# camille-004/Graph-HSCN

Hardware: AMD Instinct MI355X
Metric: graphs/sec (fwd+bwd) on Peptides-func batch=128 (higher is better)
Workload: dtype f32; 1 GPU; Graph-HSCN stage C (HSCN fwd+loss+bwd) on peptides_func-shaped graphs; graphs_per_gpu=128, global_batch=128, num_clusters=16, hidden=16, layers=3, classes=10, nodes_per_gpu=20584, ll_edges_per_gpu=41900, cluster_ids=scn_untrained, virtual_nodes_per_gpu=384, vv_edges_per_gpu=772, mode=graph, engine=resident, structure_build=per-step, steps_per_graph=15, settle=0.1 s of untimed replays before the --warmup steps

## Files before the change

### graph-hscn_amd/csrc/resident_common.h

```cpp
#pragma once
#include "hscn_common.h"

namespace {

__device__ __forceinline__ float leaky(float v, float slope) { return v > 0.f ? v : v * slope; }

typedef _Float16 half_t;
typedef _Float16 half4_t __attribute__((ext_vector_type(4)));
__device__ __forceinline__ float ldf(const float* p, size_t i) { return p[i]; }
__device__ __forceinline__ float ldf(const half_t* p, size_t i) { return (float)p[i]; }
__device__ __forceinline__ float4 ldf4(const float* p, size_t i4) { return reinterpret_cast<const float4*>(p)[i4]; }
__device__ __forceinline__ float4 ldf4(const half_t* p, size_t i4) {
  const half4_t v = reinterpret_cast<const half4_t*>(p)[i4];
  return make_float4((float)v.x, (float)v.y, (float)v.z, (float)v.w);
}
__device__ __forceinline__ void stf(float* p, size_t i, float v) { p[i] = v; }
__device__ __forceinline__ void stf(half_t* p, size_t i, float v) { p[i] = (half_t)v; }
__device__ __forceinline__ void stf4(float* p, size_t i4, float4 v) { reinterpret_cast<float4*>(p)[i4] = v; }
__device__ __forceinline__ void stf4(half_t* p, size_t i4, float4 v) {
  half4_t h;
  h.x = (half_t)v.x; h.y = (half_t)v.y; h.z = (half_t)v.z; h.w = (half_t)v.w;
  reinterpret_cast<half4_t*>(p)[i4] = h;
}
__device__ __forceinline__ void stf_sc1(float* p, size_t i, float v) {
// ... 223 lines not shown
  }
  lds_barrier();
  for (int e = G.t; e < ne; e += G.nt) {
    const int k = ek[e];
    if (k < 0) continue;
    const int p = atomicAdd(&cursor[k], -1) - 1;
    tmp[rowptr[k] + p] = e;
  }
  lds_barrier();
  for (int e = G.t; e < ne; e += G.nt) {
    const int k = ek[e];
    if (k < 0) continue;
    const int s = rowptr[k], t = rowptr[k + 1];
    int rank = 0;
    for (int q = s; q < t; ++q) rank += (tmp[q] < e) ? 1 : 0;
    col[s + rank] = eo[e];
  }
  lds_barrier();
}

constexpr int ELL_D = 6;
__device__ bool build_csr_pair_ell(const int* ek, const int* eo, int ne, int nrows, int* rowptr_a, int* col_a,
                                   int* rowptr_t, int* col_t, float* dinv, int* cnt_a, int* ell_a, int* cnt_t,
                                   int* ell_t, int* ovf, int RTn, int wave, int NWn) {
  for (int e = threadIdx.x; e < ne; e += RTn) {
    const int k = ek[e], o = eo[e];
    if (k >= 0) {
      const int pa = atomicAdd(&cnt_a[k], 1), pt = atomicAdd(&cnt_t[o], 1);
      if (pa < ELL_D) ell_a[k * ELL_D + pa] = e; else ovf[0] = 1;
      if (pt < ELL_D) ell_t[o * ELL_D + pt] = e; else ovf[0] = 1;
    }
  }
  lds_barrier();
  if (ovf[0] != 0) return false;
  const int NA = NWn > 1 ? NWn / 2 : 1;
  auto rows = [&](const int* cnt, const int* ell, const int* other, int* rowptr, int* col, float* dv, int gw, int gnw) {
    const int lane = threadIdx.x & 63, gt = gw * 64 + lane, gnt = gnw * 64;
    const int per = (nrows + gnt - 1) / gnt;
    const int wb = gw * 64 * per;
    int front = 0;
    for (int j = lane; j < wb && j < nrows; j += 64) front += cnt[j];
    front = __builtin_amdgcn_readlane(wave_incl_scan(front), 63);
    const int b = gt * per;
    int s = 0;
    for (int i = 0; i < per; ++i)
      if (b + i < nrows) s += cnt[b + i];
    int run = front + wave_incl_scan(s) - s;
    for (int i = 0; i < per; ++i) {
      const int r = b + i;
      if (r >= nrows) break;
      const int c = cnt[r];
      int ev[ELL_D];
#pragma unroll
      for (int j = 0; j < ELL_D; ++j) ev[j] = j < c ? ell[r * ELL_D + j] : 0x7fffffff;
      int ov[ELL_D];
#pragma unroll
      for (int j = 0; j < ELL_D; ++j) ov[j] = other[j < c ? ev[j] : 0];
#pragma unroll
      for (int j = 0; j < ELL_D; ++j) {
        int rank = 0;
#pragma unroll
        for (int m = 0; m < ELL_D; ++m) rank += ev[m] < ev[j] ? 1 : 0;
        if (j < c) col[run + rank] = ov[j];
      }
      rowptr[r] = run;
      if (dv) dv[r] = c > 0 ? 1.0f / sqrtf((float)c) : 0.f;
      run += c;
      if (r == nrows - 1) rowptr[nrows] = run;
    }
    if (nrows == 0 && gt == 0) rowptr[0] = 0;
  };
  if (NWn == 1) {
    rows(cnt_a, ell_a, eo, rowptr_a, col_a, dinv, 0, 1);
    rows(cnt_t, ell_t, ek, rowptr_t, col_t, nullptr, 0, 1);
  } else if (wave < NA) {
    rows(cnt_a, ell_a, eo, rowptr_a, col_a, dinv, wave, NA);
  } else {
    rows(cnt_t, ell_t, ek, rowptr_t, col_t, nullptr, wave - NA, NWn - NA);
  }
  lds_barrier();
  return true;
}

__device__ bool build_ell16_pair(const int* ek, const int* eo, int ne, int nrows, uint4* rec_a, uint4* rec_t, float* dinv,
                                 int* cnt_a, int* ell_a, int* cnt_t, int* ell_t, int* ovf, int RTn) {
  for (int e = threadIdx.x; e < ne; e += RTn) {
    const int k = ek[e], o = eo[e];
    if (k >= 0) {
      const int pa = atomicAdd(&cnt_a[k], 1), pt = atomicAdd(&cnt_t[o], 1);
      if (pa < ELL_D) ell_a[k * ELL_D + pa] = e; else ovf[0] = 1;
      if (pt < ELL_D) ell_t[o * ELL_D + pt] = e; else ovf[0] = 1;
    }
  }
  lds_barrier();
  if (ovf[0] != 0) return false;
  for (int idx = threadIdx.x; idx < 2 * nrows; idx += RTn) {
    const bool tside = idx >= nrows;
    const int r = tside ? idx - nrows : idx;
    const int* cnt = tside ? cnt_t : cnt_a;
    const int* ell = tside ? ell_t : ell_a;
    const int* other = tside ? ek : eo;
    const int c = cnt[r];
    int ev[ELL_D], ov[ELL_D];
#pragma unroll
    for (int j = 0; j < ELL_D; ++j) ev[j] = j < c ? ell[r * ELL_D + j] : 0x7fffffff;
#pragma unroll
    for (int j = 0; j < ELL_D; ++j) ov[j] = other[j < c ? ev[j] : 0];
    unsigned id[ELL_D];
#pragma unroll
    for (int j = 0; j < ELL_D; ++j) id[j] = (unsigned)r;
#pragma unroll
    for (int j = 0; j < ELL_D; ++j) {
      int rank = 0;
#pragma unroll
      for (int m = 0; m < ELL_D; ++m) rank += ev[m] < ev[j] ? 1 : 0;
#pragma unroll
      for (int q = 0; q < ELL_D; ++q)
        if (j < c && rank == q) id[q] = (unsigned)ov[j];
    }
    const uint4 rec = make_uint4(id[0] | (id[1] << 16), id[2] | (id[3] << 16), id[4] | (id[5] << 16),
                                 (unsigned)r | ((unsigned)c << 16));
    (tside ? rec_t : rec_a)[r] = rec;
    if (!tside && dinv) dinv[r] = c > 0 ? 1.0f / sqrtf((float)c) : 0.f;
  }
  lds_barrier();
  return true;
}

constexpr int CSR_MULTISPLIT_BARRIERS = 5;
__device__ void build_csr_multisplit_lds(const int* ek, const int* eo, int ne, int nrows, int* rowptr, int* col,
                                         int* cnt, int* tmp, int* wsum, const Grp& G) {
  const int nchunk = (ne + 63) >> 6;
  const int lane = threadIdx.x & 63;
  for (int i = G.t; i < nrows * nchunk; i += G.nt) cnt[i] = 0;
  lds_barrier();
  for (int c = G.w; c < nchunk; c += G.nw) {
    const int e = c * 64 + lane;
    const int k = e < ne ? ek[e] : -1;
    unsigned long long todo = __ballot(k >= 0);
    int rank = 0;
    while (todo) {
      const int leader = __ffsll((long long)todo) - 1;
      const int k0 = __builtin_amdgcn_readlane(k, leader);
      const unsigned long long m = __ballot(k == k0);
      if (k == k0) rank = __popcll(m & ((1ull << lane) - 1ull));
      if (lane == leader) cnt[k0 * nchunk + c] = __popcll(m);
      todo &= ~m;
    }
    if (e < ne) tmp[e] = rank;
  }
  lds_barrier();
  scan_inclusive_lds(cnt, nrows * nchunk, wsum, G);
  for (int r = G.t; r <= nrows; r += G.nt) rowptr[r] = (r * nchunk > 0) ? cnt[r * nchunk - 1] : 0;
  for (int e = G.t; e < ne; e += G.nt) {
    const int k = ek[e];
    if (k < 0) continue;
    const int idx = k * nchunk + (e >> 6);
    const int base = idx > 0 ? cnt[idx - 1] : 0;
    col[base + tmp[e]] = eo[e];
  }
  lds_barrier();
}

__device__ __forceinline__ void dinv_from_rowptr(const int* rowptr, int n, float* dinv, const Grp& G) {
  for (int i = G.t; i < n; i += G.nt) {
    const int d = rowptr[i + 1] - rowptr[i];
    dinv[i] = d > 0 ? 1.0f / sqrtf((float)d) : 0.f;
  }
}


template <bool ACQ>
__device__ __forceinline__ bool wait_published(const uint32_t* word, uint32_t want, int32_t* flag) {
  bool ok = true;
  if ((threadIdx.x & 63) == 0) {
    unsigned spins = 0;
// ... 74 lines not shown
```

### graph-hscn_amd/csrc/resident_kernels.h

```cpp
#pragma once
#include "hscn_common.h"
#include "resident_common.h"
#include <cstdio>

namespace {

constexpr int RT_MAX = 1024;
constexpr int MAXL = 8;

struct LayerP {
  const float *W_ll, *b_ll, *W_vv, *b_vv, *W_src, *W_dst, *att_src, *att_dst, *b_gat;
};

struct StepVCaps {
  static constexpr int N = 448, V = 32, EVV = V * (V + 1) / 2;
};

struct StepLCaps {
  static constexpr int N = 448, ELL = 1024, L = 3, C = 16;
};

struct FwdArgs {
  const float* x_local;
  const float* x_virtual;
// ... 141 lines not shown
      float d = 0.f;
#pragma unroll
      for (int q = 0; q < OPT; ++q) d = fmaf(acc[q], at[q], d);
#pragma unroll
      for (int off = LPR >> 1; off > 0; off >>= 1) d += __shfl_xor(d, off, 64);
      if (og == 0) a_out[i] = d;
    }
  }
}

template <int H>
__device__ void att_logits(const float* X, const float* Wt, const float* att, float* a_out, int n, const Grp& G) {
  constexpr int LPR = H / 4;
  constexpr int RPW = 64 / LPR;
  const int lane = threadIdx.x & 63, q = lane % LPR, rl = lane / LPR;
  if (G.w * RPW >= n) return;
  constexpr int P = 64 / H, OW = H / P;
  float wk = 0.f;
  {
    const int k = lane % H, part = lane / H;
#pragma unroll
    for (int o4 = 0; o4 < OW / 4; ++o4) {
      const float4 at = *reinterpret_cast<const float4*>(att + part * OW + 4 * o4);
      const float4 wr = *reinterpret_cast<const float4*>(Wt + k * H + part * OW + 4 * o4);
      wk = fmaf(at.w, wr.w, fmaf(at.z, wr.z, fmaf(at.y, wr.y, fmaf(at.x, wr.x, wk))));
    }
#pragma unroll
    for (int off = H; off < 64; off <<= 1) wk += __shfl_xor(wk, off, 64);
  }
  float w[4];
#pragma unroll
  for (int c = 0; c < 4; ++c) w[c] = __shfl(wk, 4 * q + c, 64);
  for (int i0 = G.w * RPW; i0 < n; i0 += G.nw * RPW) {
    const int i = i0 + rl;
    float d = 0.f;
    if (i < n) {
      const float4 x = *reinterpret_cast<const float4*>(X + i * H + 4 * q);
      d = fmaf(x.w, w[3], fmaf(x.z, w[2], fmaf(x.y, w[1], x.x * w[0])));
    }
#pragma unroll
    for (int off = LPR >> 1; off > 0; off >>= 1) d += __shfl_xor(d, off, 64);
    if (q == 0 && i < n) a_out[i] = d;
  }
}

template <int H, bool MASK>
__device__ void lin_mfma(const float* X, const float* Wt, float* Y, int n, const float* M, const Grp& G) {
  typedef float f32x4 __attribute__((ext_vector_type(4)));
  constexpr int TD = H / 16, KS = H / 4;
  const int lane = threadIdx.x & 63, li = lane & 15, lj = lane >> 4;
  const int ntile = (n + 15) >> 4;
  if (G.w >= ntile) return;
  float b[TD][KS];
#pragma unroll
  for (int ct = 0; ct < TD; ++ct)
#pragma unroll
    for (int s = 0; s < KS; ++s) b[ct][s] = Wt[(4 * s + lj) * H + ct * 16 + li];
  for (int rt = G.w; rt < ntile; rt += G.nw) {
    const int r0 = rt * 16;
    const bool ok = r0 + li < n;
    const float* xr = X + (r0 + li) * H + lj;
    f32x4 acc[TD];
#pragma unroll
    for (int ct = 0; ct < TD; ++ct) acc[ct] = f32x4{0.f, 0.f, 0.f, 0.f};
#pragma unroll
    for (int s = 0; s < KS; ++s) {
      const float a = ok ? xr[4 * s] : 0.f;
#pragma unroll
      for (int ct = 0; ct < TD; ++ct) acc[ct] = __builtin_amdgcn_mfma_f32_16x16x4f32(a, b[ct][s], acc[ct], 0, 0, 0);
    }
#pragma unroll
    for (int ct = 0; ct < TD; ++ct)
#pragma unroll
      for (int r = 0; r < 4; ++r) {
        const int row = r0 + lj * 4 + r;
        if (row < n) {
          const int idx = row * H + ct * 16 + li;
          Y[idx] = MASK ? (M[idx] > 0.f ? acc[ct][r] : 0.f) : acc[ct][r];
        }
      }
  }
}

template <int H, typename TS, bool E16 = false>
__device__ void gcn_fused(const int* rowptr, const int* col, const float* dinv, const float* X, const float* Wt,
                          const float* bias, float* Y, TS* __restrict__ gout, int n, const Grp& G,
                          float* pool_part = nullptr, float* pos_part = nullptr) {
  typedef float f32x4 __attribute__((ext_vector_type(4)));
  constexpr int TD = H / 16, KS = H / 4;
  const int lane = threadIdx.x & 63, li = lane & 15, lj = lane >> 4;
  const int ntile = (n + 15) >> 4;
  if (G.w >= ntile) {
    if (pool_part && lj == 0) {
#pragma unroll
      for (int ct = 0; ct < TD; ++ct) {
        pool_part[ct * 16 + li] = 0.f;
        if (pos_part) pos_part[ct * 16 + li] = 0.f;
      }
    }
    return;
  }
  float ps[TD], pc[TD];
#pragma unroll
  for (int ct = 0; ct < TD; ++ct) { ps[ct] = 0.f; pc[ct] = 0.f; }
  float b[TD][KS], bia[TD];
#pragma unroll
  for (int ct = 0; ct < TD; ++ct) {
    bia[ct] = bias[ct * 16 + li];
#pragma unroll
    for (int s = 0; s < KS; ++s) b[ct][s] = Wt[(KS * lj + s) * H + ct * 16 + li];
  }
  const float* xq = X + KS * lj;
  auto finish = [&](int rt_, const float (&z)[KS]) {
    const int r0 = rt_ * 16;
    f32x4 acc[TD];
#pragma unroll
    for (int ct = 0; ct < TD; ++ct) acc[ct] = f32x4{0.f, 0.f, 0.f, 0.f};
#pragma unroll
    for (int s = 0; s < KS; ++s)
#pragma unroll
      for (int ct = 0; ct < TD; ++ct) acc[ct] = __builtin_amdgcn_mfma_f32_16x16x4f32(z[s], b[ct][s], acc[ct], 0, 0, 0);
#pragma unroll
    for (int ct = 0; ct < TD; ++ct)
#pragma unroll
      for (int r = 0; r < 4; ++r) {
        const int row = r0 + lj * 4 + r;
        if (row < n) {
          const int idx = row * H + ct * 16 + li;
          const float v = rnd<TS>(fmaxf(acc[ct][r] + bia[ct], 0.f));
          Y[idx] = v;
          if (gout) stf(gout, (size_t)idx, v);
          ps[ct] += v;
          pc[ct] += v > 0.f ? 1.f : 0.f;
        }
      }
  };
  for (int rt = G.w; rt < ntile; rt += G.nw) {
    const int i = rt * 16 + li;
    float z[KS];
#pragma unroll
    for (int s = 0; s < KS; ++s) z[s] = 0.f;
    if (E16) {
      if (i < n) {
        const uint4 rec = reinterpret_cast<const uint4*>(rowptr)[i];
        const float di = dinv[i];
        const int c = (int)(rec.w >> 16);
        const int jr[8] = {(int)(rec.x & 0xffffu), (int)(rec.x >> 16), (int)(rec.y & 0xffffu), (int)(rec.y >> 16),
                           (int)(rec.z & 0xffffu), (int)(rec.z >> 16), (int)(rec.w & 0xffffu), (int)(rec.w & 0xffffu)};
#pragma unroll
        for (int p = 0; p < 8; p += 4) {
          if (p < c) {
            float w[4];
#pragma unroll
            for (int u = 0; u < 4; ++u) w[u] = p + u < c ? dinv[jr[p + u]] * di : 0.f;
#pragma unroll
            for (int q = 0; q < KS / 4; ++q) {
              float4 v[4];
#pragma unroll
              for (int u = 0; u < 4; ++u) v[u] = *reinterpret_cast<const float4*>(xq + jr[p + u] * H + 4 * q);
#pragma unroll
              for (int u = 0; u < 4; ++u) {
                z[4 * q + 0] = fmaf(w[u], v[u].x, z[4 * q + 0]);
                z[4 * q + 1] = fmaf(w[u], v[u].y, z[4 * q + 1]);
                z[4 * q + 2] = fmaf(w[u], v[u].z, z[4 * q + 2]);
                z[4 * q + 3] = fmaf(w[u], v[u].w, z[4 * q + 3]);
              }
            }
          }
        }
      }
    } else if (i < n) {
      const int s0 = rowptr[i], t0 = rowptr[i + 1];
      const float di = dinv[i];
      for (int p = s0; p < t0; p += 4) {
        int j[4];
        float w[4];
#pragma unroll
        for (int u = 0; u < 4; ++u) j[u] = col[p + u < t0 ? p + u : t0 - 1];
#pragma unroll
        for (int u = 0; u < 4; ++u) w[u] = p + u < t0 ? dinv[j[u]] * di : 0.f;
#pragma unroll
        for (int q = 0; q < KS / 4; ++q) {
          float4 v[4];
#pragma unroll
          for (int u = 0; u < 4; ++u) v[u] = *reinterpret_cast<const float4*>(xq + j[u] * H + 4 * q);
#pragma unroll
          for (int u = 0; u < 4; ++u) {
            z[4 * q + 0] = fmaf(w[u], v[u].x, z[4 * q + 0]);
            z[4 * q + 1] = fmaf(w[u], v[u].y, z[4 * q + 1]);
            z[4 * q + 2] = fmaf(w[u], v[u].z, z[4 * q + 2]);
            z[4 * q + 3] = fmaf(w[u], v[u].w, z[4 * q + 3]);
          }
        }
      }
    }
    finish(rt, z);
  }
  if (pool_part) {
#pragma unroll
    for (int ct = 0; ct < TD; ++ct) {
      float t = ps[ct];
      t += __shfl_xor(t, 16, 64);
      t += __shfl_xor(t, 32, 64);
      if (lj == 0) pool_part[ct * 16 + li] = t;
      if (pos_part) {
        float c = pc[ct];
        c += __shfl_xor(c, 16, 64);
        c += __shfl_xor(c, 32, 64);
        if (lj == 0) pos_part[ct * 16 + li] = c;
      }
    }
  }
}

template <int H>
struct Blk {
  static constexpr int OPT = H <= 16 ? 2 : 1;
};

template <int H, typename TS = float>
__device__ void agg_gcn_lds(const int* rowptr, const int* col, const float* dr, const float* dc,
                            const float* Hin, const float* bias, float* Out, int n, int relu,
                            TS* __restrict__ gout , const Grp& G) {
  constexpr int LPR = H / 4;
  const int RPB = G.nt / LPR;
  const int rl = G.t / LPR, f = (G.t % LPR) * 4;
  float4 b = make_float4(0.f, 0.f, 0.f, 0.f);
  if (bias) b = *reinterpret_cast<const float4*>(bias + f);
  for (int i = rl; i < n; i += RPB) {
    const int s = rowptr[i], t = rowptr[i + 1];
    const float di = dr[i];
    float4 a = make_float4(0.f, 0.f, 0.f, 0.f);
    for (int p = s; p < t; ++p) {
      const int j = col[p];
      const float w = mul_rn(dc[j], di);
      const float4 v = *reinterpret_cast<const float4*>(Hin + j * H + f);
      a.x = add_rn(a.x, mul_rn(w, v.x));
      a.y = add_rn(a.y, mul_rn(w, v.y));
      a.z = add_rn(a.z, mul_rn(w, v.z));
      a.w = add_rn(a.w, mul_rn(w, v.w));
    }
    a.x += b.x; a.y += b.y; a.z += b.z; a.w += b.w;
    if (relu) {
      a.x = fmaxf(a.x, 0.f); a.y = fmaxf(a.y, 0.f); a.z = fmaxf(a.z, 0.f); a.w = fmaxf(a.w, 0.f);
    }
    if (gout) { a.x = rnd<TS>(a.x); a.y = rnd<TS>(a.y); a.z = rnd<TS>(a.z); a.w = rnd<TS>(a.w); }
    *reinterpret_cast<float4*>(Out + i * H + f) = a;
    if (gout) stf4(gout, ((size_t)i * H + f) >> 2, a);
  }
}

struct FwdLayout {
  size_t xa, bh, xva, xvb, zs, a_s, a_d, sc, dinv, dinv_v, wt, headw, part, vec;
  size_t rowptr, col, rowptr_lv, col_lv, rowptr_vv, col_vv, cursorA, tmpA, cursorB, tmpB, wsum;
  size_t rowptr_t, col_t, cursorT, tmpT, cursorV, tmpV;
  size_t ck_tab, ck_first, ck_arrive, gpart;
  size_t ek_ll, eo_ll, ek_lv, eo_lv, ek_vv, eo_vv, total;
};
__host__ __device__ inline FwdLayout fwd_layout(int H, int C, int max_n, int max_v, int max_ell, int max_evv,
                                                int db, int exp) {
  FwdLayout Y;
  size_t o = 0;
  auto take = [&](size_t n) { size_t r = o; o += (n + 3) & ~(size_t)3; return r; };
  Y.xa = take((size_t)max_n * H);
  size_t xq = Y.xa;
  const size_t xend = Y.xa + (size_t)max_n * H;
  auto scratch = [&](size_t n) {
    const size_t need = (n + 3) & ~(size_t)3;
    if (xq + need <= xend) { const size_t r = xq; xq += need; return r; }
    return take(n);
  };
  const size_t stage = (size_t)2 * (((size_t)max_ell + 3) / 4 * 4 + ((size_t)max_n + 3) / 4 * 4 +
                                    ((size_t)max_evv + 3) / 4 * 4);
  const size_t two = (size_t)max_n * H;
  const size_t region = take(two > stage ? two : stage);
  Y.bh = region;
  {
    size_t p = region;
    auto sub = [&](size_t n) { size_t r = p; p += (n + 3) & ~(size_t)3; return r; };
    Y.ek_ll = sub(max_ell); Y.eo_ll = sub(max_ell);
    Y.ek_lv = sub(max_n);   Y.eo_lv = sub(max_n);
    Y.ek_vv = sub(max_evv); Y.eo_vv = sub(max_evv);
  }
  Y.xva = take((size_t)max_v * H);
  Y.xvb = take((size_t)max_v * H);
  Y.zs = take(max_v ? (size_t)(RT_MAX / 64) * H : 0);
  Y.a_s = take(max_n);
  Y.a_d = take(max_v);
  Y.sc = take(max_n);
  Y.dinv = take(max_n);
  Y.dinv_v = take(max_v);
  Y.wt = take((size_t)(db ? 2 : 1) * (4 * H * H + 5 * H));
  Y.headw = take((size_t)H * H + H + (size_t)C * H + C);
  Y.part = take((size_t)(RT_MAX / 64) * H);
  Y.vec = take(128);
// ... 1842 lines not shown
```

### graph-hscn_amd/csrc/resident_step.h

```cpp

struct StepArgs {
  const float* x_local;
  const int64_t *ll_src, *ll_dst;
  const int32_t *lptr, *eptr_ll;
  const float* W_ll[MAXL];
  const float* b_ll[MAXL];
  const float *W1, *b1, *W2, *b2;
  const float* target;
  float *pred, *score;
  float* partials;
  float* acts;
  uint32_t* ready;
  const uint32_t* epoch;
  const int32_t *pre_rp_d, *pre_col_d, *pre_rp_s, *pre_col_s;
  const float* pre_dinv;
  int32_t* flag;
  int64_t N;
  int F, L, C, head_act, max_n, max_ell, P, Pn, loss_kind;
  float inv_count;
  int B;
};

struct StepLayout {
  size_t A, dinv, wt, headw, part, vec, red, rowptr, col, rowptr_t, col_t, wsum, total;
// ... 150 lines not shown
#pragma unroll
  for (int i = 0; i < XPT; ++i) {
    const int idx = threadIdx.x + i * RT;
    const int r = idx / H, k = idx - r * H;
    const bool ok = idx < n * H && k < F;
    xr[i] = 0.f;
    if (wbase + i * RT < n * H) {
      const float t = ldf(xl_g, ok ? (size_t)(n0 + r) * F + k : 0);
      xr[i] = ok ? t : 0.f;
    }
  }
  float wr[WPT];
  const int WTOT = L * WL;
#pragma unroll
  for (int i = 0; i < WPT; ++i) {
    const int d = threadIdx.x + i * RT;
    const int l = d / WL, q = d - l * WL;
    const int fin = l == 0 ? F : H;
    wr[i] = 0.f;
    if (wbase + i * RT < WTOT) {
      const bool inb = d < WTOT;
      const int ll = inb ? l : 0;
      const bool isb = q >= H * H;
      const int k = q / H, o = q - k * H;
      const bool ok = inb && (isb || k < fin);
      const float* src = isb ? A.b_ll[ll] + (q - H * H) : A.W_ll[ll] + (ok ? o * fin + k : 0);
      const float t = *(ok ? src : A.b_ll[0]);
      wr[i] = ok ? t : 0.f;
    }
  }
  const int HT = H * H + H + C * H + C;
  auto haddr = [&](int idx) -> const float* {
    if (idx < H * H) return A.W1 + idx;
    idx -= H * H;
    if (idx < H) return A.b1 + idx;
    idx -= H;
    if (idx < C * H) return A.W2 + idx;
    idx -= C * H;
    if (idx < C) return A.b2 + idx;
    idx -= C;
    return A.target + (size_t)g * C + (idx < C ? idx : 0);
  };
  const int HTT = HT + C;
  float hw0 = *haddr((int)threadIdx.x < HTT ? (int)threadIdx.x : 0);
  float hw1 = *haddr((int)threadIdx.x + RT < HTT ? (int)threadIdx.x + RT : 0);
  if (pre) {
#pragma unroll
    for (int i = 0; i < EPT; ++i) {
      const int e = threadIdx.x + i * RT;
      if (e <= n) { rowptr[e] = prd[i]; rowptr_t[e] = prs[i]; }
      if (e < n) dinv[e] = pdv[i];
      if (e < ne) { col[e] = pcd[i]; col_t[e] = pcs[i]; }
    }
    for (int e = threadIdx.x + EPT * RT; e <= n; e += RT) {
      rowptr[e] = A.pre_rp_d[(size_t)n0 + g + e];
      rowptr_t[e] = A.pre_rp_s[(size_t)n0 + g + e];
      if (e < n) dinv[e] = A.pre_dinv[(size_t)n0 + e];
    }
    for (int e = threadIdx.x + EPT * RT; e < ne; e += RT) {
      col[e] = A.pre_col_d[(size_t)e0 + e];
      col_t[e] = A.pre_col_s[(size_t)e0 + e];
    }
  } else {
    int *ek = ib + Y.ek, *eo = ib + Y.eo;
    bool bad = false;
#pragma unroll
    for (int i = 0; i < EPT; ++i) {
      const int e = threadIdx.x + i * RT;
      if (e < ne) {
        int k = (int)(rld[i] - n0), o_ = (int)(rls[i] - n0);
        if (k < 0 || k >= n || o_ < 0 || o_ >= n) { bad = true; k = -1; o_ = -1; }
        ek[e] = k; eo[e] = o_;
      }
    }
    for (int e = threadIdx.x + EPT * RT; e < ne; e += RT) {
      int k = (int)(A.ll_dst[e0 + e] - n0), o_ = (int)(A.ll_src[e0 + e] - n0);
      if (k < 0 || k >= n || o_ < 0 || o_ >= n) { bad = true; k = -1; o_ = -1; }
      ek[e] = k; eo[e] = o_;
    }
    if (bad && A.flag) atomicOr(A.flag, 2);
  }
  for (int i = threadIdx.x; i <= n; i += RT) { (ib + Y.cntA)[i] = 0; (ib + Y.cntT)[i] = 0; }
  if (threadIdx.x == 0) { (ib + Y.wsum)[0] = 0; (ib + Y.wsum)[1] = 0; (ib + Y.ovf)[0] = 0; }
  {
    float* x0 = buf(0);
#pragma unroll
    for (int i = 0; i < XPT; ++i) {
      const int idx = threadIdx.x + i * RT;
      if (idx < n * H) x0[idx] = xr[i];
    }
    for (int idx = threadIdx.x + XPT * RT; idx < n * H; idx += RT) {
      const int r = idx / H, k = idx - r * H;
      x0[idx] = k < F ? ldf(xl_g, (size_t)(n0 + r) * F + k) : 0.f;
    }
#pragma unroll
    for (int i = 0; i < WPT; ++i) {
      const int d = threadIdx.x + i * RT;
      if (d < WTOT) wt[d] = wr[i];
    }
    for (int d = threadIdx.x + WPT * RT; d < WTOT; d += RT) {
      const int l = d / WL, q = d - l * WL;
      const int fin = l == 0 ? F : H;
      const int k = q / H, o = q - k * H;
      wt[d] = q >= H * H ? A.b_ll[l][q - H * H] : (k < fin ? A.W_ll[l][o * fin + k] : 0.f);
    }
    if ((int)threadIdx.x < HTT) headw[threadIdx.x] = hw0;
    if ((int)threadIdx.x + RT < HTT) headw[threadIdx.x + RT] = hw1;
    for (int idx = threadIdx.x + 2 * RT; idx < HTT; idx += RT) headw[idx] = *haddr(idx);
  }
  lds_barrier();
  STAMP(1);
  bool e16 = false;
  if (!pre) {
    bool low;
    if (H == 16) {
      low = build_ell16_pair(ib + Y.ek, ib + Y.eo, ne, n, reinterpret_cast<uint4*>(ib + Y.rowptr),
                             reinterpret_cast<uint4*>(ib + Y.recT), dinv, ib + Y.cntA, ib + Y.ellA, ib + Y.cntT,
                             ib + Y.ellT, ib + Y.ovf, RT);
      e16 = low;
    } else {
      low = build_csr_pair_ell(ib + Y.ek, ib + Y.eo, ne, n, rowptr, col, rowptr_t, col_t, dinv, ib + Y.cntA,
                               ib + Y.ellA, ib + Y.cntT, ib + Y.ellT, ib + Y.ovf, RT, wave, NW);
    }
    if (!low) {
      const int NA = NW / 2 > 0 ? NW / 2 : 1;
      const bool inB = wave >= NA && NW > 1;
      if (NW == 1) {
        build_csr_lds(ib + Y.ek, ib + Y.eo, ne, n, rowptr, col, ib + Y.cursorA, ib + Y.tmpA, ALL, true);
        build_csr_lds(ib + Y.eo, ib + Y.ek, ne, n, rowptr_t, col_t, ib + Y.cursorT, ib + Y.tmpT, ALL, true);
        dinv_from_rowptr(rowptr, n, dinv, ALL);
      } else if (!inB) {
        const Grp GA{(int)threadIdx.x, NA * 64, wave, NA};
        build_csr_lds(ib + Y.ek, ib + Y.eo, ne, n, rowptr, col, ib + Y.cursorA, ib + Y.tmpA, GA, true);
        dinv_from_rowptr(rowptr, n, dinv, GA);
      } else {
        const Grp GB{(int)threadIdx.x - NA * 64, (NW - NA) * 64, wave - NA, NW - NA};
        build_csr_lds(ib + Y.eo, ib + Y.ek, ne, n, rowptr_t, col_t, ib + Y.cursorT, ib + Y.tmpT, GB, true);
      }
    }
  }
  lds_barrier();
  STAMP(3);
  const bool hand = acts_g != nullptr && L >= 2;
  constexpr int NE = NW >= 16 ? 2 : 1;
  const int NC = hand && NW > 1 ? NW - NE : NW;
  const Grp GC{(int)threadIdx.x, NC * 64, wave, NC};
  auto export_rows = [&](const float* src, TS* dst) {
    typedef unsigned int u32x4 __attribute__((ext_vector_type(4)));
    typedef unsigned int u32x2 __attribute__((ext_vector_type(2)));
    const int cnt = n * (H / 4);
    const __amdgpu_buffer_rsrc_t rs = __builtin_amdgcn_make_buffer_rsrc(dst, 0, cnt * 4 * (int)sizeof(TS), 0x00020000);
    const int ew = NW > 1 ? wave - NC : 0, nes = NW > 1 ? NE : 1;
    for (int i0 = ew * 64 + lane; i0 < cnt; i0 += 4 * nes * 64) {
      float4 v[4];
#pragma unroll
      for (int u = 0; u < 4; ++u) {
        const int i = i0 + u * nes * 64;
        v[u] = reinterpret_cast<const float4*>(src)[i < cnt ? i : i0];
      }
#pragma unroll
      for (int u = 0; u < 4; ++u) {
        const int i = i0 + u * nes * 64;
        if (i >= cnt) continue;
        if constexpr (sizeof(TS) == 4) {
          u32x4 w = {__float_as_uint(v[u].x), __float_as_uint(v[u].y), __float_as_uint(v[u].z), __float_as_uint(v[u].w)};
          __builtin_amdgcn_raw_buffer_store_b128(w, rs, i * 16, 0, 16 );
        } else {
          half4_t h;
          h.x = (half_t)v[u].x; h.y = (half_t)v[u].y; h.z = (half_t)v[u].z; h.w = (half_t)v[u].w;
          u32x2 w;
          __builtin_memcpy(&w, &h, 8);
          __builtin_amdgcn_raw_buffer_store_b64(w, rs, i * 8, 0, 16 );
        }
      }
    }
  };
  int* exp_cnt = ib + Y.wsum + 1;
  auto raise = [&](int upto) {
    asm volatile("s_waitcnt vmcnt(0)" ::: "memory");
    int last = 1;
    if (NE > 1 && NW > 1) {
      int arrived = 0;
      if (lane == 0) arrived = __hip_atomic_fetch_add(exp_cnt, 1, __ATOMIC_ACQ_REL, __HIP_MEMORY_SCOPE_WORKGROUP);
      arrived = __builtin_amdgcn_readfirstlane(arrived);
      last = (arrived % NE) == NE - 1;
    }
    if (last && A.ready && lane == 0)
      __hip_atomic_store(A.ready + g, ep8 + (uint32_t)upto, __ATOMIC_RELAXED, __HIP_MEMORY_SCOPE_AGENT);
  };
  for (int l = 0; l < L; ++l) {
    STAMP(4 + l);
    float* pool_w = l == L - 1 ? partp + wave * H : nullptr;
    float* pos_w = l == L - 1 ? partp + NW * H + wave * H : nullptr;
    if (wave < NC) {
      if (e16) gcn_fused<H, TS, true>(rowptr, col, dinv, buf(l), wt + l * WL, wt + l * WL + H * H, buf(l + 1), (TS*)nullptr, n, GC, pool_w, pos_w);
      else gcn_fused<H, TS, false>(rowptr, col, dinv, buf(l), wt + l * WL, wt + l * WL + H * H, buf(l + 1), (TS*)nullptr, n, GC, pool_w, pos_w);
    } else if (hand) {
      if (pool_w && lane < H) { pool_w[lane] = 0.f; if (pos_w) pos_w[lane] = 0.f; }
      if (l >= 2) raise(l - 1);
      if (l >= 1) export_rows(buf(l), acts_g + ((size_t)(l - 1) * A.N + n0) * H);
    }
    lds_barrier();
  }
  if (hand && NW == 1) {
    for (int l = 1; l < L; ++l) export_rows(buf(l), acts_g + ((size_t)(l - 1) * A.N + n0) * H);
    raise(L - 1);
  }
  STAMP(12);
  float* aL = buf(L);
  float* pol = vec;
  float* zz = vec + 64;
  float* gz = vec + 128;
  float* gpool = vec + 192;
  float* gpn = vec + 256;
  const float* W1l = headw;
  const float* b1l = headw + H * H;
  const float* W2l = b1l + H;
  const float* b2l = W2l + C * H;
  const float* tgl = b2l + C;
  float* gpl = headw + HT + C;
  float* ltl = gpl + C;
  const bool fast_head = H == 16 && C <= 16;
  if (threadIdx.x < 64) {
    const float cnt = (float)(n > 0 ? n : 1);
    if (fast_head) {
      constexpr int HH = H <= 16 ? H : 16;
      const bool lh = lane < HH, lc = lane < C;
      const int lk = lh ? lane : 0, lcc = lc ? lane : 0;
      float pw[NW], w1r[HH], w1c[HH], w2r[HH], w2c[16];
#pragma unroll
      for (int w = 0; w < NW; ++w) pw[w] = partp[w * H + lk];
#pragma unroll
      for (int k4 = 0; k4 < HH / 4; ++k4) {
        const float4 a = *reinterpret_cast<const float4*>(W1l + lk * H + 4 * k4);
        w1r[4 * k4] = a.x; w1r[4 * k4 + 1] = a.y; w1r[4 * k4 + 2] = a.z; w1r[4 * k4 + 3] = a.w;
        const float4 b = *reinterpret_cast<const float4*>(W2l + lcc * H + 4 * k4);
        w2r[4 * k4] = b.x; w2r[4 * k4 + 1] = b.y; w2r[4 * k4 + 2] = b.z; w2r[4 * k4 + 3] = b.w;
      }
#pragma unroll
      for (int o = 0; o < HH; ++o) w1c[o] = W1l[o * H + lk];
#pragma unroll
      for (int c = 0; c < 16; ++c) w2c[c] = c < C ? W2l[c * H + lk] : 0.f;
      const float bb1 = b1l[lk], bb2 = b2l[lcc], tgt = tgl[lcc];
      float s = 0.f;
#pragma unroll
      for (int w = 0; w < NW; ++w) s += pw[w];
      const float polv = s / cnt;
      const float zv = apply_act(row_dot<HH>(polv, w1r, 0.f) + bb1, A.head_act);
      const float pc = row_dot<HH>(zv, w2r, 0.f) + bb2;
      float lt, sg, gg;
      criterion_elem(A.loss_kind, pc, tgt, A.inv_count, lt, sg, gg);
      if (lc) {
        A.pred[(size_t)g * C + lane] = pc;
        if (A.score) A.score[(size_t)g * C + lane] = sg;
      }
      lt = lc ? lt : 0.f;
      gg = lc ? gg : 0.f;
      const float sl = row_seq_sum<16>(lt, 0.f);
      const float gzv = row_dot<16>(gg, w2c, 0.f) * act_grad_from_output(zv, A.head_act);
      const float gpa = row_dot<HH>(gzv, w1c, 0.f);
      if (lh) { pol[lane] = polv; zz[lane] = zv; gz[lane] = gzv; gpool[lane] = gpa; gpn[lane] = gpa / cnt; }
      if (lc) gpl[lane] = gg;
      if (lane == 0) part[A.Pn] = sl;
    } else {
    if (lane < H) {
      float s = 0.f;
#pragma unroll
      for (int w = 0; w < NW; ++w) s += partp[w * H + lane];
      s = s / cnt;
      pol[lane] = s;
    }
    __builtin_amdgcn_fence(__ATOMIC_SEQ_CST, "wavefront");
    if (lane < H) {
      float a1 = 0.f;
      const float4* wrow = reinterpret_cast<const float4*>(W1l + lane * H);
#pragma unroll
      for (int k4 = 0; k4 < H / 4; ++k4) {
        const float4 w4 = wrow[k4];
        const float4 p4 = *reinterpret_cast<const float4*>(pol + 4 * k4);
        a1 = fmaf(p4.x, w4.x, a1);
        a1 = fmaf(p4.y, w4.y, a1);
        a1 = fmaf(p4.z, w4.z, a1);
        a1 = fmaf(p4.w, w4.w, a1);
      }
      a1 += b1l[lane];
      a1 = apply_act(a1, A.head_act);
      zz[lane] = a1;
    }
    __builtin_amdgcn_fence(__ATOMIC_SEQ_CST, "wavefront");
    for (int c = lane; c < C; c += 64) {
      float a2 = 0.f;
      const float4* wrow = reinterpret_cast<const float4*>(W2l + c * H);
#pragma unroll
      for (int k4 = 0; k4 < H / 4; ++k4) {
        const float4 w4 = wrow[k4];
        const float4 z4 = *reinterpret_cast<const float4*>(zz + 4 * k4);
        a2 = fmaf(z4.x, w4.x, a2);
        a2 = fmaf(z4.y, w4.y, a2);
        a2 = fmaf(z4.z, w4.z, a2);
        a2 = fmaf(z4.w, w4.w, a2);
      }
      const float pc = a2 + b2l[c];
      float lt, sg, gg;
      criterion_elem(A.loss_kind, pc, tgl[c], A.inv_count, lt, sg, gg);
      gpl[c] = gg;
      ltl[c] = lt;
      A.pred[(size_t)g * C + c] = pc;
      if (A.score) A.score[(size_t)g * C + c] = sg;
    }
    __builtin_amdgcn_fence(__ATOMIC_SEQ_CST, "wavefront");
    if (lane < H) {
      float acc = 0.f;
      for (int c = 0; c < C; ++c) acc = fmaf(gpl[c], W2l[c * H + lane], acc);
      gz[lane] = acc * act_grad_from_output(zz[lane], A.head_act);
    }
    __builtin_amdgcn_fence(__ATOMIC_SEQ_CST, "wavefront");
    if (lane < H) {
      float acc = 0.f;
#pragma unroll
      for (int o = 0; o < H; ++o) acc = fmaf(gz[o], W1l[o * H + lane], acc);
      gpool[lane] = acc;
      gpn[lane] = acc / cnt;
    }
    }
  }
  lds_barrier();
  STAMP(13);
  if (hand && wave >= NC && NW > 1) raise(L - 1);

  int off_head = 0;
  for (int l = 0; l < L; ++l) off_head += H * (l == 0 ? F : H) + H;
  const int oW1 = off_head, ob1 = oW1 + H * H, oW2 = ob1 + H, ob2 = oW2 + C * H;
  for (int idx = threadIdx.x; idx < C * H; idx += RT) {
    const int c = idx / H, k = idx - c * H;
    part[oW2 + idx] = gpl[c] * zz[k];
  }
  for (int c = threadIdx.x; c < C; c += RT) part[ob2 + c] = gpl[c];
  if (!fast_head && threadIdx.x == RT - 64) {
    float sl = 0.f;
    for (int c = 0; c < C; ++c) sl += ltl[c];
    part[A.Pn] = sl;
  }
  for (int idx = threadIdx.x; idx < H * H; idx += RT) {
    const int o = idx / H, k = idx - o * H;
    part[oW1 + idx] = gz[o] * pol[k];
  }
  if (threadIdx.x < H) part[ob1 + threadIdx.x] = gz[threadIdx.x];
  float* G = aL;
  float* GH = L >= 2 ? buf(0) : buf(2);
  if constexpr (H != 16) {
    const float cnt = (float)(n > 0 ? n : 1);
    for (int idx = threadIdx.x; idx < n * H; idx += RT) G[idx] = G[idx] > 0.f ? gpool[idx % H] / cnt : 0.f;
  }
  STAMP(14);
  float* bred = partp;
  constexpr int GW_TD = H / 16, GW_NT = GW_TD * GW_TD;
  constexpr int GW_TPP = GW_NT < NW ? GW_NT : NW, GW_RG = NW / GW_TPP;
  constexpr bool GW1 = GW_NT <= NW;
  auto fold_gw = [&](int t0, int oW_, int fin_) {
    for (int idx = threadIdx.x; idx < GW_TPP * 256; idx += RT) {
      const int t_ = t0 + idx / 256, e_ = idx & 255;
      if (t_ < GW_NT) {
        float s_ = 0.f;
#pragma unroll
        for (int r = 0; r < GW_RG; ++r) s_ += red[(r * GW_TPP + idx / 256) * 256 + e_];
        const int oo = (t_ / GW_TD) * 16 + (e_ >> 4), kk = (t_ % GW_TD) * 16 + (e_ & 15);
        if (kk < fin_) part[oW_ + oo * fin_ + kk] = s_;
      }
    }
  };
  int pend_oW = -1, pend_fin = 0;
  int off = off_head;
  if constexpr (H == 16) {
    typedef float f32x4 __attribute__((ext_vector_type(4)));
    int* fold_cnt = ib + Y.wsum;
    constexpr int NFW = NW < 4 ? NW : 4;
    float* Gc = aL;
    const int li = lane & 15, lj = lane >> 4;
    const int ntile = (n + 15) >> 4;
    int pend_ob = 0;
    const float4 gq4 = *reinterpret_cast<const float4*>(gpn + 4 * lj);
    auto gl4 = [](const float4 a, const float4 q) {
      return make_float4(a.x > 0.f ? q.x : 0.f, a.y > 0.f ? q.y : 0.f, a.z > 0.f ? q.z : 0.f, a.w > 0.f ? q.w : 0.f);
    };
    for (int it = 0, l = L - 1; l >= 0; --l, ++it) {
      const int fin = l == 0 ? F : H;
      off -= H * fin + H;
      const int oW = off, ob = off + H * fin;
      float* bredw = bred + (it % 3) * NW * H;
      float* bredn = bred + ((it + 1) % 3) * NW * H;
      float bsum = 0.f;
      if (it > 0) lds_barrier();
      if (pend_oW >= 0) {
        const int ft = (int)threadIdx.x - (RT - NFW * 64);
        if (ft >= 0) {
          const int e_ = ft & 255;
          float s_ = 0.f;
#pragma unroll
          for (int r = 0; r < NW; ++r) s_ += red[r * 256 + e_];
          const int oo = e_ >> 4, kk = e_ & 15;
          if (kk < pend_fin) part[pend_oW + oo * pend_fin + kk] = s_;
        }
        if ((int)threadIdx.x >= RT - H) {
          const int c_ = (int)threadIdx.x - (RT - H);
          const float* bp = bred + ((it - 1) % 3) * NW * H;
          float sb = 0.f;
#pragma unroll
          for (int w = 0; w < NW; ++w) sb += bp[w * H + c_];
          part[pend_ob + c_] = sb;
        }
        if (wave >= NW - NFW) {
          __builtin_amdgcn_fence(__ATOMIC_RELEASE, "workgroup");
          if (lane == 0) __hip_atomic_fetch_add(fold_cnt, 1, __ATOMIC_RELAXED, __HIP_MEMORY_SCOPE_WORKGROUP);
        }
      }
      if (it == 0) {
        if (lane < H) bredw[wave * H + lane] = (partp + NW * H)[wave * H + lane] * gpn[lane];
      }
      float* Xl = buf(l);
      const float* Wl = wt + l * WL;
      float bw[4];
#pragma unroll
      for (int s = 0; s < 4; ++s) bw[s] = l > 0 ? Wl[li * H + 4 * lj + s] : 0.f;
      f32x4 accw = {0.f, 0.f, 0.f, 0.f};
      float* sc = (it == 0 ? red : aL) + wave * 256;
      const float* gq = Gc + 4 * lj;
      auto finish = [&](int rt_, const float4 z) {
        const int r0 = rt_ * 16;
        __builtin_amdgcn_fence(__ATOMIC_SEQ_CST, "wavefront");
        *reinterpret_cast<float4*>(sc + li * 16 + 4 * lj) = z;
        f32x4 acc = {0.f, 0.f, 0.f, 0.f};
        if (l > 0) {
          acc = __builtin_amdgcn_mfma_f32_16x16x4f32(z.x, bw[0], acc, 0, 0, 0);
          acc = __builtin_amdgcn_mfma_f32_16x16x4f32(z.y, bw[1], acc, 0, 0, 0);
          acc = __builtin_amdgcn_mfma_f32_16x16x4f32(z.z, bw[2], acc, 0, 0, 0);
          acc = __builtin_amdgcn_mfma_f32_16x16x4f32(z.w, bw[3], acc, 0, 0, 0);
        }
        __builtin_amdgcn_fence(__ATOMIC_SEQ_CST, "wavefront");
#pragma unroll
        for (int c = 0; c < 4; ++c) {
          const int row = r0 + 4 * c + lj;
          const float av = sc[(4 * c + lj) * 16 + li];
          const float bv = row < n ? Xl[row * H + li] : 0.f;
          accw = __builtin_amdgcn_mfma_f32_16x16x4f32(av, bv, accw, 0, 0, 0);
        }
        if (l > 0) {
          __builtin_amdgcn_fence(__ATOMIC_SEQ_CST, "wavefront");
#pragma unroll
          for (int r = 0; r < 4; ++r) {
            const int row = r0 + lj * 4 + r;
            if (row < n) {
              const int idx = row * H + li;
              const float gnew = Xl[idx] > 0.f ? acc[r] : 0.f;
              Xl[idx] = gnew;
              bsum += gnew;
            }
          }
        }
      };
      for (int rt = wave; rt < ntile; rt += NW) {
        const int i = rt * 16 + li;
        float4 z = make_float4(0.f, 0.f, 0.f, 0.f);
        if (e16) {
          if (i < n) {
            const uint4 rec = reinterpret_cast<const uint4*>(ib + Y.recT)[i];
            const float di = dinv[i];
            const int c = (int)(rec.w >> 16);
            const int jr[8] = {(int)(rec.x & 0xffffu), (int)(rec.x >> 16), (int)(rec.y & 0xffffu), (int)(rec.y >> 16),
                               (int)(rec.z & 0xffffu), (int)(rec.z >> 16), (int)(rec.w & 0xffffu), (int)(rec.w & 0xffffu)};
#pragma unroll
            for (int p = 0; p < 8; p += 4) {
              if (p < c) {
                float ww[4];
                float4 vv[4];
#pragma unroll
                for (int u = 0; u < 4; ++u) {
                  ww[u] = mul_rn(dinv[jr[p + u]], di);
                  vv[u] = *reinterpret_cast<const float4*>(gq + jr[p + u] * H);
                  if (it == 0) vv[u] = gl4(vv[u], gq4);
                }
#pragma unroll
                for (int u = 0; u < 4; ++u) {
                  if (p + u < c) {
                    z.x = fmaf(ww[u], vv[u].x, z.x); z.y = fmaf(ww[u], vv[u].y, z.y);
                    z.z = fmaf(ww[u], vv[u].z, z.z); z.w = fmaf(ww[u], vv[u].w, z.w);
                  }
                }
              }
            }
          }
        } else if (i < n) {
          const int s0 = rowptr_t[i], t0 = rowptr_t[i + 1];
          const float di = dinv[i];
          for (int p = s0; p < t0; p += 4) {
            int jj[4];
            float ww[4];
            float4 vv[4];
#pragma unroll
            for (int u = 0; u < 4; ++u) jj[u] = col_t[p + u < t0 ? p + u : t0 - 1];
#pragma unroll
            for (int u = 0; u < 4; ++u) {
              ww[u] = mul_rn(dinv[jj[u]], di);
              vv[u] = *reinterpret_cast<const float4*>(gq + jj[u] * H);
              if (it == 0) vv[u] = gl4(vv[u], gq4);
            }
#pragma unroll
            for (int u = 0; u < 4; ++u) {
              if (p + u < t0) {
                z.x = fmaf(ww[u], vv[u].x, z.x); z.y = fmaf(ww[u], vv[u].y, z.y);
                z.z = fmaf(ww[u], vv[u].z, z.z); z.w = fmaf(ww[u], vv[u].w, z.w);
              }
            }
          }
        }
        finish(rt, z);
      }
      if (it > 0) {
        while (__hip_atomic_load(fold_cnt, __ATOMIC_RELAXED, __HIP_MEMORY_SCOPE_WORKGROUP) < it * NFW)
          __builtin_amdgcn_s_sleep(1);
        __builtin_amdgcn_fence(__ATOMIC_ACQUIRE, "workgroup");
      }
      __builtin_amdgcn_fence(__ATOMIC_SEQ_CST, "wavefront");
#pragma unroll
      for (int r = 0; r < 4; ++r) red[wave * 256 + (lj * 4 + r) * 16 + li] = accw[r];
      if (l > 0) {
        bsum += __shfl_xor(bsum, 16, 64);
        bsum += __shfl_xor(bsum, 32, 64);
        if (lj == 0) bredn[wave * H + li] = bsum;
      }
      pend_oW = oW; pend_fin = fin; pend_ob = ob;
      Gc = Xl;
      STAMP(16 + 3 * l);
    }
    lds_barrier();
    fold_gw(0, pend_oW, pend_fin);
    if (threadIdx.x < H) {
      const float* bp = bred + ((L - 1) % 3) * NW * H;
      float sb = 0.f;
#pragma unroll
      for (int w = 0; w < NW; ++w) sb += bp[w * H + threadIdx.x];
      part[pend_ob + threadIdx.x] = sb;
    }
    STAMP(61);
    return;
  }
  for (int l = L - 1; l >= 0; --l) {
    const int fin = l == 0 ? F : H;
    off -= H * fin + H;
    const int oW = off, ob = off + H * fin;
    lds_barrier();
    if (GW1 && pend_oW >= 0) fold_gw(0, pend_oW, pend_fin);
    const bool reload = l == 0 && L >= 2;
    float* X = reload ? buf(1) : buf(l);
    float xq[XPT];
    if (reload) {
#pragma unroll
      for (int i = 0; i < XPT; ++i) {
        const int idx = threadIdx.x + i * RT;
        const int r = idx / H, k = idx - r * H;
        xq[i] = (idx < n * H && k < fin) ? ldf(xl_g, (size_t)(n0 + r) * fin + k) : 0.f;
      }
    }
    {
      constexpr int LQ = H / 4;
      constexpr int SQ = 64 / LQ;
      const int slot = lane / LQ, f = (lane % LQ) * 4;
      float4 acc = make_float4(0.f, 0.f, 0.f, 0.f);
      for (int i = wave * SQ + slot; i < n; i += NW * SQ) {
        const float4 v = *reinterpret_cast<const float4*>(G + i * H + f);
        acc.x += v.x; acc.y += v.y; acc.z += v.z; acc.w += v.w;
      }
#pragma unroll
      for (int o_ = 32; o_ >= 16 && o_ >= LQ; o_ >>= 1) {
        acc.x += __shfl_xor(acc.x, o_, 64);
        acc.y += __shfl_xor(acc.y, o_, 64);
        acc.z += __shfl_xor(acc.z, o_, 64);
        acc.w += __shfl_xor(acc.w, o_, 64);
      }
      if (LQ <= 8) {
        acc.x = row_ror_add<8>(acc.x); acc.y = row_ror_add<8>(acc.y);
        acc.z = row_ror_add<8>(acc.z); acc.w = row_ror_add<8>(acc.w);
      }
      if (LQ <= 4) {
        acc.x = row_ror_add<4>(acc.x); acc.y = row_ror_add<4>(acc.y);
        acc.z = row_ror_add<4>(acc.z); acc.w = row_ror_add<4>(acc.w);
      }
      if (slot == 0) *reinterpret_cast<float4*>(bred + wave * H + f) = acc;
    }
    agg_gcn_lds<H, float>(rowptr_t, col_t, dinv, dinv, G, nullptr, GH, n, 0, (float*)nullptr, ALL);
    if (reload) {
#pragma unroll
      for (int i = 0; i < XPT; ++i) {
        const int idx = threadIdx.x + i * RT;
        if (idx < n * H) X[idx] = xq[i];
      }
      for (int idx = threadIdx.x + XPT * RT; idx < n * H; idx += RT) {
        const int r = idx / H, k = idx - r * H;
        X[idx] = k < fin ? ldf(xl_g, (size_t)(n0 + r) * fin + k) : 0.f;
      }
    }
    lds_barrier();
    STAMP(16 + 3 * l);
    if (threadIdx.x < H) {
      float sb = 0.f;
#pragma unroll
      for (int w = 0; w < NW; ++w) sb += bred[w * H + threadIdx.x];
      part[ob + threadIdx.x] = sb;
    }
    {
      typedef float f32x4 __attribute__((ext_vector_type(4)));
      constexpr int TD = GW_TD, NT = GW_NT, TPP = GW_TPP, RG = GW_RG;
      const int li = lane & 15, lj = lane >> 4;
// ... 103 lines not shown
```

Baseline: 5.195 million graphs/s.

## Prefetch GCN weights and ELL row records ahead of barriers in resident step

Splits gcn_fused into operand-staging and body pieces so each wave can load its layer weights, bias and first-tile ELL neighbour weights before the barrier that precedes the layer. The next layer's operands are staged right after the current one finishes. Feature/weight parking is moved into the structure build, between the atomic ELL fill and its barrier, and a redundant barrier is dropped after a successful build. Backward weights and transposed row records are also preloaded before the head and between layers. The aim is to hide global/LDS load latency behind barriers, at the cost of more registers held live.

```diff
diff --git a/graph-hscn_amd/csrc/resident_common.h b/graph-hscn_amd/csrc/resident_common.h
--- a/graph-hscn_amd/csrc/resident_common.h
+++ b/graph-hscn_amd/csrc/resident_common.h
@@ -329,8 +329,10 @@
   return true;
 }
 
-__device__ bool build_ell16_pair(const int* ek, const int* eo, int ne, int nrows, uint4* rec_a, uint4* rec_t, float* dinv,
-                                 int* cnt_a, int* ell_a, int* cnt_t, int* ell_t, int* ovf, int RTn) {
+template <typename Mid>
+__device__ __forceinline__ bool build_ell16_pair(const int* ek, const int* eo, int ne, int nrows, uint4* rec_a, uint4* rec_t,
+                                                 float* dinv, int* cnt_a, int* ell_a, int* cnt_t, int* ell_t, int* ovf,
+                                                 int RTn, Mid&& mid) {
   for (int e = threadIdx.x; e < ne; e += RTn) {
     const int k = ek[e], o = eo[e];
     if (k >= 0) {
@@ -339,6 +341,7 @@
       if (pt < ELL_D) ell_t[o * ELL_D + pt] = e; else ovf[0] = 1;
     }
   }
+  mid();
   lds_barrier();
   if (ovf[0] != 0) return false;
   for (int idx = threadIdx.x; idx < 2 * nrows; idx += RTn) {
diff --git a/graph-hscn_amd/csrc/resident_kernels.h b/graph-hscn_amd/csrc/resident_kernels.h
--- a/graph-hscn_amd/csrc/resident_kernels.h
+++ b/graph-hscn_amd/csrc/resident_kernels.h
@@ -247,12 +247,51 @@
   }
 }
 
+template <int H>
+struct GcnOps {
+  float b[H / 16][H / 4], bia[H / 16];
+};
+struct GcnRow {
+  uint4 rec;
+  float w[ELL_D];
+};
+template <int H>
+__device__ __forceinline__ void gcn_stage_ops(GcnOps<H>& O, const float* Wt, const float* bias) {
+  constexpr int TD = H / 16, KS = H / 4;
+  const int lane = threadIdx.x & 63, li = lane & 15, lj = lane >> 4;
+#pragma unroll
+  for (int ct = 0; ct < TD; ++ct) {
+    O.bia[ct] = bias[ct * 16 + li];
+#pragma unroll
+    for (int s = 0; s < KS; ++s) O.b[ct][s] = Wt[(KS * lj + s) * H + ct * 16 + li];
+  }
+}
+template <bool RN>
+__device__ __forceinline__ void gcn_stage_row(GcnRow& R, const uint4* recs, const float* dinv, int i, int n) {
+  R.rec = make_uint4(0u, 0u, 0u, 0u);
+#pragma unroll
+  for (int u = 0; u < ELL_D; ++u) R.w[u] = 0.f;
+  if (i < n) {
+    R.rec = recs[i];
+    const float di = dinv[i];
+    const int c = (int)(R.rec.w >> 16);
+    const int jr[ELL_D] = {(int)(R.rec.x & 0xffffu), (int)(R.rec.x >> 16), (int)(R.rec.y & 0xffffu),
+                           (int)(R.rec.y >> 16), (int)(R.rec.z & 0xffffu), (int)(R.rec.z >> 16)};
+#pragma unroll
+    for (int u = 0; u < ELL_D; ++u) {
+      const float dj = dinv[jr[u]];
+      R.w[u] = u < c ? (RN ? mul_rn(dj, di) : dj * di) : 0.f;
+    }
+  }
+}
+
 template <int H, typename TS, bool E16 = false>
-__device__ void gcn_fused(const int* rowptr, const int* col, const float* dinv, const float* X, const float* Wt,
-                          const float* bias, float* Y, TS* __restrict__ gout, int n, const Grp& G,
-                          float* pool_part = nullptr, float* pos_part = nullptr) {
+__device__ __forceinline__ void gcn_body(const int* rowptr, const int* col, const float* dinv, const float* X,
+                                         const GcnOps<H>& O, const GcnRow* row0, float* Y, TS* __restrict__ gout, int n,
+                                         const Grp& G, float* pool_part = nullptr, float* pos_part = nullptr) {
   typedef float f32x4 __attribute__((ext_vector_type(4)));
   constexpr int TD = H / 16, KS = H / 4;
+  static_assert(ELL_D == 6, "a row record holds six neighbour ids");
   const int lane = threadIdx.x & 63, li = lane & 15, lj = lane >> 4;
   const int ntile = (n + 15) >> 4;
   if (G.w >= ntile) {
@@ -268,13 +307,8 @@
   float ps[TD], pc[TD];
 #pragma unroll
   for (int ct = 0; ct < TD; ++ct) { ps[ct] = 0.f; pc[ct] = 0.f; }
-  float b[TD][KS], bia[TD];
-#pragma unroll
-  for (int ct = 0; ct < TD; ++ct) {
-    bia[ct] = bias[ct * 16 + li];
-#pragma unroll
-    for (int s = 0; s < KS; ++s) b[ct][s] = Wt[(KS * lj + s) * H + ct * 16 + li];
-  }
+  const auto& b = O.b;
+  const auto& bia = O.bia;
   const float* xq = X + KS * lj;
   auto finish = [&](int rt_, const float (&z)[KS]) {
     const int r0 = rt_ * 16;
@@ -306,18 +340,21 @@
 #pragma unroll
     for (int s = 0; s < KS; ++s) z[s] = 0.f;
     if (E16) {
+      GcnRow R;
+      if (row0 && rt == G.w) R = *row0;
+      else gcn_stage_row<false>(R, reinterpret_cast<const uint4*>(rowptr), dinv, i, n);
       if (i < n) {
-        const uint4 rec = reinterpret_cast<const uint4*>(rowptr)[i];
-        const float di = dinv[i];
+        const uint4 rec = R.rec;
         const int c = (int)(rec.w >> 16);
         const int jr[8] = {(int)(rec.x & 0xffffu), (int)(rec.x >> 16), (int)(rec.y & 0xffffu), (int)(rec.y >> 16),
                            (int)(rec.z & 0xffffu), (int)(rec.z >> 16), (int)(rec.w & 0xffffu), (int)(rec.w & 0xffffu)};
+        const float wr[8] = {R.w[0], R.w[1], R.w[2], R.w[3], R.w[4], R.w[5], 0.f, 0.f};
 #pragma unroll
         for (int p = 0; p < 8; p += 4) {
           if (p < c) {
             float w[4];
 #pragma unroll
-            for (int u = 0; u < 4; ++u) w[u] = p + u < c ? dinv[jr[p + u]] * di : 0.f;
+            for (int u = 0; u < 4; ++u) w[u] = wr[p + u];
 #pragma unroll
             for (int q = 0; q < KS / 4; ++q) {
               float4 v[4];
@@ -376,6 +413,15 @@
       }
     }
   }
+}
+
+template <int H, typename TS, bool E16 = false>
+__device__ void gcn_fused(const int* rowptr, const int* col, const float* dinv, const float* X, const float* Wt,
+                          const float* bias, float* Y, TS* __restrict__ gout, int n, const Grp& G,
+                          float* pool_part = nullptr, float* pos_part = nullptr) {
+  GcnOps<H> O;
+  if (G.w < ((n + 15) >> 4)) gcn_stage_ops<H>(O, Wt, bias);
+  gcn_body<H, TS, E16>(rowptr, col, dinv, X, O, nullptr, Y, gout, n, G, pool_part, pos_part);
 }
 
 template <int H>
diff --git a/graph-hscn_amd/csrc/resident_step.h b/graph-hscn_amd/csrc/resident_step.h
--- a/graph-hscn_amd/csrc/resident_step.h
+++ b/graph-hscn_amd/csrc/resident_step.h
@@ -256,7 +256,10 @@
   }
   for (int i = threadIdx.x; i <= n; i += RT) { (ib + Y.cntA)[i] = 0; (ib + Y.cntT)[i] = 0; }
   if (threadIdx.x == 0) { (ib + Y.wsum)[0] = 0; (ib + Y.wsum)[1] = 0; (ib + Y.ovf)[0] = 0; }
-  {
+  static_assert(YF.ek >= YF.A + YF.bufw && YF.cntA >= YF.A + 2 * YF.bufw && YF.dinv >= YF.A + YF.NB * YF.bufw &&
+                    YF.wt > YF.dinv && YF.headw > YF.wt && YF.rowptr > YF.headw,
+                "features / weights are parked while the structure build owns A[1] and A[2]");
+  auto park = [&]() {
     float* x0 = buf(0);
 #pragma unroll
     for (int i = 0; i < XPT; ++i) {
@@ -281,21 +284,25 @@
     if ((int)threadIdx.x < HTT) headw[threadIdx.x] = hw0;
     if ((int)threadIdx.x + RT < HTT) headw[threadIdx.x + RT] = hw1;
     for (int idx = threadIdx.x + 2 * RT; idx < HTT; idx += RT) headw[idx] = *haddr(idx);
-  }
+  };
+  constexpr bool park_in_build = H == 16;
+  if (pre || !park_in_build) park();
   lds_barrier();
   STAMP(1);
   bool e16 = false;
+  bool built = false;
   if (!pre) {
     bool low;
-    if (H == 16) {
+    if constexpr (H == 16) {
       low = build_ell16_pair(ib + Y.ek, ib + Y.eo, ne, n, reinterpret_cast<uint4*>(ib + Y.rowptr),
                              reinterpret_cast<uint4*>(ib + Y.recT), dinv, ib + Y.cntA, ib + Y.ellA, ib + Y.cntT,
-                             ib + Y.ellT, ib + Y.ovf, RT);
+                             ib + Y.ellT, ib + Y.ovf, RT, park);
       e16 = low;
     } else {
       low = build_csr_pair_ell(ib + Y.ek, ib + Y.eo, ne, n, rowptr, col, rowptr_t, col_t, dinv, ib + Y.cntA,
                                ib + Y.ellA, ib + Y.cntT, ib + Y.ellT, ib + Y.ovf, RT, wave, NW);
     }
+    built = low;
     if (!low) {
       const int NA = NW / 2 > 0 ? NW / 2 : 1;
       const bool inB = wave >= NA && NW > 1;
@@ -313,7 +320,7 @@
       }
     }
   }
-  lds_barrier();
+  if (!built) lds_barrier();
   STAMP(3);
   const bool hand = acts_g != nullptr && L >= 2;
   constexpr int NE = NW >= 16 ? 2 : 1;
@@ -362,17 +369,46 @@
     if (last && A.ready && lane == 0)
       __hip_atomic_store(A.ready + g, ep8 + (uint32_t)upto, __ATOMIC_RELAXED, __HIP_MEMORY_SCOPE_AGENT);
   };
+  const int ntile_f = (n + 15) >> 4;
+  const bool fwd_own = wave < NC && wave < ntile_f;
+  GcnOps<H> fops;
+  GcnRow frow;
+  if (fwd_own) {
+    gcn_stage_ops<H>(fops, wt, wt + H * H);
+    if constexpr (H == 16)
+      if (e16) gcn_stage_row<false>(frow, reinterpret_cast<const uint4*>(rowptr), dinv, wave * 16 + (lane & 15), n);
+  }
+  const int HW = NC - 1;
+  GcnRow brow;
+  float bw[4];
+  auto stage_bwd = [&](int l_) {
+    const float* Wl_ = wt + l_ * WL;
+#pragma unroll
+    for (int s = 0; s < 4; ++s) bw[s] = l_ > 0 ? Wl_[(lane & 15) * H + 4 * (lane >> 4) + s] : 0.f;
+  };
+  auto stage_bwd_row = [&]() {
+    if constexpr (H == 16)
+      if (e16 && wave < ntile_f)
+        gcn_stage_row<true>(brow, reinterpret_cast<const uint4*>(ib + Y.recT), dinv, wave * 16 + (lane & 15), n);
+  };
   for (int l = 0; l < L; ++l) {
     STAMP(4 + l);
     float* pool_w = l == L - 1 ? partp + wave * H : nullptr;
     float* pos_w = l == L - 1 ? partp + NW * H + wave * H : nullptr;
     if (wave < NC) {
-      if (e16) gcn_fused<H, TS, true>(rowptr, col, dinv, buf(l), wt + l * WL, wt + l * WL + H * H, buf(l + 1), (TS*)nullptr, n, GC, pool_w, pos_w);
-      else gcn_fused<H, TS, false>(rowptr, col, dinv, buf(l), wt + l * WL, wt + l * WL + H * H, buf(l + 1), (TS*)nullptr, n, GC, pool_w, pos_w);
+      if (e16) gcn_body<H, TS, true>(rowptr, col, dinv, buf(l), fops, &frow, buf(l + 1), (TS*)nullptr, n, GC, pool_w, pos_w);
+      else gcn_body<H, TS, false>(rowptr, col, dinv, buf(l), fops, nullptr, buf(l + 1), (TS*)nullptr, n, GC, pool_w, pos_w);
+      if (l + 1 < L && fwd_own) gcn_stage_ops<H>(fops, wt + (l + 1) * WL, wt + (l + 1) * WL + H * H);
     } else if (hand) {
       if (pool_w && lane < H) { pool_w[lane] = 0.f; if (pos_w) pos_w[lane] = 0.f; }
       if (l >= 2) raise(l - 1);
       if (l >= 1) export_rows(buf(l), acts_g + ((size_t)(l - 1) * A.N + n0) * H);
+    }
+    if constexpr (H == 16) {
+      if (l == L - 1 && wave != HW) {
+        stage_bwd_row();
+        stage_bwd(L - 1);
+      }
     }
     lds_barrier();
   }
@@ -395,7 +431,7 @@
   float* gpl = headw + HT + C;
   float* ltl = gpl + C;
   const bool fast_head = H == 16 && C <= 16;
-  if (threadIdx.x < 64) {
+  if (wave == HW) {
     const float cnt = (float)(n > 0 ? n : 1);
     if (fast_head) {
       constexpr int HH = H <= 16 ? H : 16;
@@ -501,6 +537,9 @@
   lds_barrier();
   STAMP(13);
   if (hand && wave >= NC && NW > 1) raise(L - 1);
+  if constexpr (H == 16) {
+    if (wave == HW) { stage_bwd_row(); stage_bwd(L - 1); }
+  }
 
   int off_head = 0;
   for (int l = 0; l < L; ++l) off_head += H * (l == 0 ? F : H) + H;
@@ -592,10 +631,6 @@
         if (lane < H) bredw[wave * H + lane] = (partp + NW * H)[wave * H + lane] * gpn[lane];
       }
       float* Xl = buf(l);
-      const float* Wl = wt + l * WL;
-      float bw[4];
-#pragma unroll
-      for (int s = 0; s < 4; ++s) bw[s] = l > 0 ? Wl[li * H + 4 * lj + s] : 0.f;
       f32x4 accw = {0.f, 0.f, 0.f, 0.f};
       float* sc = (it == 0 ? red : aL) + wave * 256;
       const float* gq = Gc + 4 * lj;
@@ -636,9 +671,12 @@
         const int i = rt * 16 + li;
         float4 z = make_float4(0.f, 0.f, 0.f, 0.f);
         if (e16) {
+          GcnRow R;
+          if (rt == wave) R = brow;
+          else gcn_stage_row<true>(R, reinterpret_cast<const uint4*>(ib + Y.recT), dinv, i, n);
           if (i < n) {
-            const uint4 rec = reinterpret_cast<const uint4*>(ib + Y.recT)[i];
-            const float di = dinv[i];
+            const uint4 rec = R.rec;
+            const float wr8[8] = {R.w[0], R.w[1], R.w[2], R.w[3], R.w[4], R.w[5], 0.f, 0.f};
             const int c = (int)(rec.w >> 16);
             const int jr[8] = {(int)(rec.x & 0xffffu), (int)(rec.x >> 16), (int)(rec.y & 0xffffu), (int)(rec.y >> 16),
                                (int)(rec.z & 0xffffu), (int)(rec.z >> 16), (int)(rec.w & 0xffffu), (int)(rec.w & 0xffffu)};
@@ -649,7 +687,7 @@
                 float4 vv[4];
 #pragma unroll
                 for (int u = 0; u < 4; ++u) {
-                  ww[u] = mul_rn(dinv[jr[p + u]], di);
+                  ww[u] = wr8[p + u];
                   vv[u] = *reinterpret_cast<const float4*>(gq + jr[p + u] * H);
                   if (it == 0) vv[u] = gl4(vv[u], gq4);
                 }
@@ -702,6 +740,7 @@
         bsum += __shfl_xor(bsum, 32, 64);
         if (lj == 0) bredn[wave * H + li] = bsum;
       }
+      if (l > 0) stage_bwd(l - 1);
       pend_oW = oW; pend_fin = fin; pend_ob = ob;
       Gc = Xl;
       STAMP(16 + 3 * l);
```

Result: slower. 4.976 million graphs/s (-4.2%).
